# baajur/sda

Hardware: AMD Instinct MI355X
Metric: clerk share-combine GB/s + packed-Shamir shares/s at 1M-dim, 1/2/4/8 GPUs (higher is better)
Workload: dtype int64; 1 GPU; AdditiveSharing clerk combine, 10k participations x 1M-dim i64 shares per GPU (BASELINE.json configs[1]); participations_per_gpu=10000, dim=1000000, modulus=2147482801, parallelism=participation split x1, exact=combiner.rs:16-28 recurrence, bit-exact, buffers=torch.empty

## Files before the change

sda_amd/csrc/engine.cpp:

```cpp
#include "../../include/sda_engine.h"

#include <dlfcn.h>
#include <hip/hip_runtime.h>
#include <rccl/rccl.h>
#include <stdarg.h>
#include <stdio.h>
#include <stdlib.h>
#include <string.h>

#include <algorithm>
#include <map>
#include <mutex>
#include <string>
#include <thread>
#include <vector>

#include "host_pack.h"
#include "kernels.h"

struct sda_engine {
    int device = 0;
    hipStream_t stream = nullptr;
    void* work = nullptr;
    size_t work_bytes = 0;
    void* stage = nullptr;
    size_t stage_bytes = 0;
    sda::DeviceTable gen_tab;
    void* gen_log = nullptr;
    size_t gen_log_bytes = 0;
    bool gen_log_used = false;
    void* gen32_tmp = nullptr;
    size_t gen32_tmp_bytes = 0;
    void* codec_work = nullptr;
    size_t codec_work_bytes = 0;
    void* codec_mat = nullptr;
    size_t codec_mat_bytes = 0;
    void* pipe = nullptr;
    size_t pipe_bytes = 0;
    sda::DeviceTable rev_tab;
    void* snap = nullptr;
    size_t snap_bytes = 0;
    hipStream_t last_stream = nullptr;
    hipEvent_t order_ev = nullptr;
    bool order_ok = true;
    unsigned long long* rej_host = nullptr;
    hipStream_t copy_stream = nullptr;
    hipEvent_t h2d_done[2] = {nullptr, nullptr}, tile_free[2] = {nullptr, nullptr};
    void* hs_pin = nullptr;
    size_t hs_pin_bytes = 0;
    void* hs_dev = nullptr;
    size_t hs_dev_bytes = 0;
    uint64_t hs_tiles32 = 0, hs_tiles64 = 0, hs_bytes_h2d = 0;
    std::vector<sda_engine*> sub;
    void** comms = nullptr;
};

namespace {

thread_local std::string g_last_error;

thread_local sda_engine* t_call_h = nullptr;
thread_local hipStream_t t_call_s = nullptr;

void end_call() {
    if (t_call_h) {
        t_call_h->order_ok = hipEventRecord(t_call_h->order_ev, t_call_s) == hipSuccess;
        t_call_h = nullptr;
    }
}

thread_local int t_depth = 0;
struct CallScope {
    CallScope() { ++t_depth; }
    ~CallScope() {
        if (--t_depth == 0) end_call();
    }
    CallScope(const CallScope&) = delete;
    CallScope& operator=(const CallScope&) = delete;
};
#define SDA_ENTRY CallScope sda_call_scope_

sda_status fail(sda_status st, const char* fmt, ...) {
    char buf[512];
    va_list ap;
    va_start(ap, fmt);
    vsnprintf(buf, sizeof(buf), fmt, ap);
    va_end(ap);
    g_last_error = buf;
    return st;
}

sda_status ok() {
    g_last_error.clear();
    return SDA_OK;
}

#define HIP_TRY(expr)                                                                              \
    do {                                                                                           \
        hipError_t _e = (expr);                                                                    \
        if (_e != hipSuccess) {                                                                    \
            (void)hipGetLastError();                                                               \
            return fail(_e == hipErrorOutOfMemory ? SDA_ERR_OUT_OF_MEMORY : SDA_ERR_DEVICE,        \
                        "%s failed: %s (%s:%d)", #expr, hipGetErrorString(_e), __FILE__, __LINE__); \
        }                                                                                          \
    } while (0)

constexpr size_t kScratchHbmMin = (size_t)256 << 20;
bool scratch_hbm(size_t bytes) {
    static const bool on = [] {
        const char* e = getenv("SDA_SCRATCH_HBM");
        return e && atoi(e) == 1;
    }();
    return on && bytes >= kScratchHbmMin;
}
bool hbm_owned(void* p);
void hbm_engine_opened(int device);
bool hbm_engine_closed(int device);

void dev_free(void* p) {
    if (!p) return;
    if (hbm_owned(p)) (void)sda_hbm_free(p);
    else (void)hipFree(p);
}

sda_status dev_alloc(void** p, size_t bytes) {
    *p = nullptr;
    if (scratch_hbm(bytes)) {
        int d = 0;
        HIP_TRY(hipGetDevice(&d));
        return sda_hbm_alloc(d, bytes, p);
    }
    HIP_TRY(hipMalloc(p, bytes));
    return SDA_OK;
}

sda_status ensure(void** buf, size_t* have, size_t need) {
    if (need <= *have) return SDA_OK;
    dev_free(*buf);
    *buf = nullptr;
    *have = 0;
    size_t want = need + need / 4 + 4096;
    if (sda_status e = dev_alloc(buf, want)) return e;
    *have = want;
    return SDA_OK;
}

hipStream_t pick(sda_engine* h, void* stream) {
    hipStream_t s = static_cast<hipStream_t>(stream);
    if (s != h->last_stream) {
        if (!h->order_ok || hipStreamWaitEvent(s, h->order_ev, 0) != hipSuccess) (void)hipDeviceSynchronize();
        h->last_stream = s;
    }
    t_call_h = h;
    t_call_s = s;
    return s;
}

bool is_pow(uint64_t x, uint64_t b) {
    if (x < 1) return false;
    while (x % b == 0) x /= b;
    return x == 1;
}

// ... 1602 lines not shown
                                                static_cast<int64_t*>(h->hs_dev)))
            return e;
    }
    DevArena a;
    if (sda_status e = stage(h, rup(n_idx * share_len * 8 + 8) + rup(n_masks * width * 8 + 8) + rup(outn * 8 + 8), &a))
        return e;
    int64_t* dsh = a.take<int64_t>(n_idx * share_len + 1);
    void* dmask = a.take<int64_t>(n_masks * width + 1);
    int64_t* dout = a.take<int64_t>(outn + 1);
    for (uint64_t i = 0; i < n_idx; ++i)
        if (share_len) HIP_TRY(hipMemcpyAsync(dsh + i * share_len, share_rows[i], share_len * 8, hipMemcpyHostToDevice, h->stream));
    if (ms->kind == SDA_MASKING_FULL)
        for (uint64_t i = 0; i < n_masks; ++i)
            if (width) HIP_TRY(hipMemcpyAsync(static_cast<int64_t*>(dmask) + i * width, mask_rows[i], width * 8,
                                              hipMemcpyHostToDevice, h->stream));
    if (ms->kind == SDA_MASKING_CHACHA && !seeds.empty() && !multi_mask)
        HIP_TRY(hipMemcpyAsync(dmask, seeds.data(), seeds.size() * 4, hipMemcpyHostToDevice, h->stream));
    uint64_t len = 0;
    if (sda_status e = multi_mask
                           ? recipient_pipeline(h, &full_row, h->hs_dev, 1, ms->dimension, ss, dimension, indices, dsh,
                                                n_idx, share_len, output_modulus, mode, dout, (uint64_t)-1, &len, h->stream)
                           : recipient_pipeline(h, ms, dmask, n_masks, ms->kind == SDA_MASKING_NONE ? 0 : width, ss,
                                                dimension, indices, dsh, n_idx, share_len, output_modulus, mode, dout,
                                                (uint64_t)-1, &len, h->stream))
        return e;
    if (out_cap < len) return fail(SDA_ERR_INVALID_ARGUMENT, "output buffer too small");
    if (len) HIP_TRY(hipMemcpyAsync(out, dout, len * 8, hipMemcpyDeviceToHost, h->stream));
    *out_len = len;
    return finish(h);
}

sda_status sda_participant_share_dev(sda_engine* h, const sda_masking_scheme* ms, const uint32_t* seed,
                                     uint64_t seed_words, const int64_t* full_masks, const sda_sharing_scheme* ss,
                                     const int64_t* secrets, uint64_t dimension, const int64_t* draws,
                                     int32_t mode, int64_t* shares_out, uint8_t* payload, uint64_t payload_cap,
                                     uint64_t* payload_row_bytes, void* stream) {
    SDA_ENTRY;
    if (!h || !ms || !ss || (dimension && (!secrets || !shares_out)) || (payload && !payload_row_bytes))
        return fail(SDA_ERR_INVALID_ARGUMENT, "NULL argument");
    HIP_TRY(hipSetDevice(h->device));
    hipStream_t st = pick(h, stream);
    const uint64_t D = dimension;
    const bool packed = ss->kind == SDA_SHARING_PACKED_SHAMIR;
    if (!packed && ss->kind != SDA_SHARING_ADDITIVE) return fail(SDA_ERR_INVALID_ARGUMENT, "unknown sharing scheme kind");
    if (mode != SDA_REVEAL_EXACT && mode != SDA_REVEAL_CANONICAL) return fail(SDA_ERR_INVALID_ARGUMENT, "bad mode");
    if (packed) {
        if (sda_status e = check_packed(ss)) return e;
    } else {
        if (ss->share_count == 0) return fail(SDA_ERR_PRECONDITION, "share_count - 1 underflows (additive.rs:42)");
        if (ss->modulus <= 0) return fail(SDA_ERR_PRECONDITION, "Rng.gen_range called with low >= high");
    }
    const int64_t* masked = secrets;
    bool mask_pending = false;
    int64_t* cmask = nullptr;
    uint32_t* cseed = nullptr;
    uint32_t cw = 0;
    if (ms->kind != SDA_MASKING_NONE && D) {
        if (ms->modulus <= 0) return fail(SDA_ERR_PRECONDITION, "Rng.gen_range called with low >= high");
        if (sda_status e = ensure(&h->pipe, &h->pipe_bytes, 2 * rup(D * 8) + 256)) return e;
        int64_t* dm = static_cast<int64_t*>(h->pipe);
        if (ms->kind == SDA_MASKING_FULL) {
            if (!full_masks) return fail(SDA_ERR_INVALID_ARGUMENT, "Full masking needs the drawn masks");
            HIP_TRY(sda::launch_addsub_trem(secrets, full_masks, +1, D, dm, ms->modulus, st));
        } else if (ms->kind == SDA_MASKING_CHACHA) {
            if (ms->dimension != D) return fail(SDA_ERR_PRECONDITION, "assertion failed: dimension == secrets.len()");
            const uint64_t want = (ms->seed_bitsize + 31) / 32;
            if (seed_words != want || (seed_words && !seed))
                return fail(SDA_ERR_PRECONDITION, "expected %llu seed words", (unsigned long long)want);
            int64_t* dmask = dm + rup(D * 8) / 8;
            uint32_t* dseed = reinterpret_cast<uint32_t*>(dmask + rup(D * 8) / 8);
            const uint32_t w = (uint32_t)(seed_words < 8 ? seed_words : 8);
            if (w) HIP_TRY(hipMemcpyAsync(dseed, seed, w * 4, hipMemcpyHostToDevice, st));
            const char* force = getenv("SDA_CHACHA_PATH");
            if (!sda::chacha_needs_stream_path(ms->modulus) && !(force && strcmp(force, "stream") == 0)) {
                if (sda_status e = ensure(&h->work, &h->work_bytes, sda::chacha_work_bytes(D, 0))) return e;
                HIP_TRY(sda::launch_chacha_mask_add_async(ms->modulus, D, dseed, w, secrets, dm, h->work, st,
                                                          h->rej_host));
                mask_pending = true;
            } else {
                if (sda_status e = chacha_combine(h, ms->modulus, D, dseed, w, 1, dmask, st)) return e;
                HIP_TRY(sda::launch_addsub_trem(secrets, dmask, +1, D, dm, ms->modulus, st));
            }
            cmask = dmask;
            cseed = dseed;
            cw = w;
        } else {
            return fail(SDA_ERR_INVALID_ARGUMENT, "unknown masking scheme kind");
        }
        masked = dm;
    }
    const uint64_t n = ss->share_count;
    const uint64_t B = packed ? (D + ss->secret_count - 1) / ss->secret_count : D;
    if (B && !draws) return fail(SDA_ERR_INVALID_ARGUMENT, "need the randomness draws");
    if (payload && n > 65535) return fail(SDA_ERR_UNSUPPORTED, "at most 65535 clerks");
    auto share_and_encode = [&]() -> sda_status {
        if (B) {
            if (packed) {
                if (sda_status e = ensure(&h->gen_log, &h->gen_log_bytes, sda::packed_gen_log_bytes())) return e;
                sda::PackedGenArgs ga{masked, D, 1, draws, shares_out, mode == SDA_REVEAL_CANONICAL};
                HIP_TRY(sda::launch_packed_generate(ga, (uint32_t)ss->secret_count, (uint32_t)ss->privacy_threshold,
                                                    (uint32_t)n, (uint32_t)ss->modulus, (uint32_t)ss->omega_secrets,
                                                    (uint32_t)ss->omega_shares, h->gen_tab, h->gen_log, st,
                                                    &h->gen_log_used));
            } else {
                HIP_TRY(sda::launch_additive_generate(masked, D, draws, n, shares_out, ss->modulus, st));
            }
        }
        if (payload) {
            if (sda_status e = ensure(&h->codec_work, &h->codec_work_bytes, sda::varint_encode_work_bytes(n, B)))
                return e;
            hipError_t e = sda::launch_varint_encode(shares_out, n, B, B, payload, payload_cap, h->codec_work,
                                                     payload_row_bytes, st);
            if (e == hipErrorInvalidValue) return fail(SDA_ERR_INVALID_ARGUMENT, "payload_cap too small");
            HIP_TRY(e);
        }
        return SDA_OK;
    };
    if (sda_status e = share_and_encode()) return e;
    if (mask_pending) {
        HIP_TRY(hipStreamSynchronize(st));
        if (*h->rej_host) {
            if (sda_status e = chacha_combine(h, ms->modulus, D, cseed, cw, 1, cmask, st)) return e;
            HIP_TRY(sda::launch_addsub_trem(secrets, cmask, +1, D, const_cast<int64_t*>(masked), ms->modulus, st));
            if (sda_status e = share_and_encode()) return e;
        }
    }
    return ok();
}

}

namespace {

long long env_ll(const char* name, long long dflt) {
    const char* e = getenv(name);
    return e && *e ? atoll(e) : dflt;
}

int host_threads(size_t devices = 1) {
    const long long t = env_ll("SDA_HOST_THREADS", 0);
    if (t > 0) return (int)std::min<long long>(t, 1024);
    const unsigned hc = std::thread::hardware_concurrency();
    return (int)std::max<unsigned>(1u, std::min<unsigned>(hc ? hc : 1u, 16u * (unsigned)devices));
}

uint64_t host_stage_bytes() {
    const long long mb = env_ll("SDA_HOST_STAGE_MB", 256);
    return (uint64_t)std::max<long long>(mb, 1) << 20;
}

using sda::pack_rows;
using sda::pack_rows32;

bool host_narrow() { return env_ll("SDA_HOST_NARROW", 1) != 0; }

sda_status host_stream_ensure(sda_engine* h, size_t tile_bytes, size_t acc_bytes) {
    if (!h->copy_stream) {
        HIP_TRY(hipStreamCreateWithFlags(&h->copy_stream, hipStreamNonBlocking));
        for (int b = 0; b < 2; ++b) {
            HIP_TRY(hipEventCreateWithFlags(&h->h2d_done[b], hipEventDisableTiming));
            HIP_TRY(hipEventCreateWithFlags(&h->tile_free[b], hipEventDisableTiming));
        }
    }
    if (h->hs_pin_bytes < 2 * rup(tile_bytes)) {
        if (h->hs_pin) (void)hipHostFree(h->hs_pin);
        h->hs_pin = nullptr;
        h->hs_pin_bytes = 0;
        HIP_TRY(hipHostMalloc(&h->hs_pin, 2 * rup(tile_bytes), hipHostMallocDefault));
        h->hs_pin_bytes = 2 * rup(tile_bytes);
    }
    const size_t dev_need = 2 * rup(tile_bytes) + rup(acc_bytes);
    if (h->hs_dev_bytes < dev_need) {
        dev_free(h->hs_dev);
        h->hs_dev = nullptr;
        h->hs_dev_bytes = 0;
        if (sda_status e = dev_alloc(&h->hs_dev, dev_need)) return e;
        h->hs_dev_bytes = dev_need;
    }
    return SDA_OK;
}

sda_status stream_combine_slice(sda_engine* h, int64_t m, const int64_t* const* rows, uint64_t n_rows, uint64_t lo,
                                uint64_t w, int64_t* out_host, int threads) {
    HIP_TRY(hipSetDevice(h->device));
    const uint64_t stage = host_stage_bytes();
    const bool narrow = host_narrow();
    const uint64_t wc_max = std::max<uint64_t>(2, stage / 8 / 2 * 2);
    for (uint64_t c0 = 0; c0 < w; c0 += wc_max) {
        const uint64_t wc = std::min(wc_max, w - c0);
        const uint64_t R = std::max<uint64_t>(1, stage / (wc * 8));
        const size_t tile = (size_t)(std::min(R, std::max<uint64_t>(n_rows, 1)) * wc * 8);
        if (sda_status e = host_stream_ensure(h, tile, wc * 8)) return e;
        int64_t* dt[2] = {static_cast<int64_t*>(h->hs_dev), static_cast<int64_t*>(h->hs_dev) + rup(tile) / 8};
        int64_t* acc = static_cast<int64_t*>(h->hs_dev) + 2 * rup(tile) / 8;
        int64_t* hp[2] = {static_cast<int64_t*>(h->hs_pin), static_cast<int64_t*>(h->hs_pin) + rup(tile) / 8};
        uint64_t i = 0;
        bool try32 = narrow;
        for (uint64_t r0 = 0; r0 < n_rows; r0 += R, ++i) {
            const uint64_t Ri = std::min(R, n_rows - r0);
            const int b = (int)(i & 1);
            if (i >= 2) HIP_TRY(hipEventSynchronize(h->h2d_done[b]));
            if (try32) try32 = pack_rows32(reinterpret_cast<int32_t*>(hp[b]), rows, r0, Ri, lo + c0, wc, threads);
            if (!try32) pack_rows(hp[b], rows, r0, Ri, lo + c0, wc, threads);
            const size_t bytes = (size_t)(Ri * wc * (try32 ? 4 : 8));
            if (i >= 2) HIP_TRY(hipStreamWaitEvent(h->copy_stream, h->tile_free[b], 0));
            HIP_TRY(hipMemcpyAsync(dt[b], hp[b], bytes, hipMemcpyHostToDevice, h->copy_stream));
            HIP_TRY(hipEventRecord(h->h2d_done[b], h->copy_stream));
            HIP_TRY(hipStreamWaitEvent(h->stream, h->h2d_done[b], 0));
            if (try32)
                HIP_TRY(sda::launch_combine_wide32(reinterpret_cast<const int32_t*>(dt[b]), Ri, wc, wc, acc, m,
                                                   h->stream, i > 0));
            else
                HIP_TRY(sda::launch_combine_exact(dt[b], Ri, wc, wc, acc, m, h->stream, i > 0));
            HIP_TRY(hipEventRecord(h->tile_free[b], h->stream));
            ++(try32 ? h->hs_tiles32 : h->hs_tiles64);
            h->hs_bytes_h2d += bytes;
        }
        HIP_TRY(hipMemcpyAsync(out_host + c0, acc, wc * 8, hipMemcpyDeviceToHost, h->stream));
        HIP_TRY(hipStreamSynchronize(h->stream));
    }
    return SDA_OK;
}

size_t n_devices(const sda_engine* h) { return h->sub.empty() ? 1 : h->sub.size(); }

template <typename F>
sda_status for_devices(sda_engine* h, F fn) {
    const size_t G = n_devices(h);
    if (G == 1) return fn(0);
    std::vector<sda_status> st(G, SDA_OK);
    std::vector<std::string> msg(G);
    std::vector<std::thread> ts;
    for (size_t g = 1; g < G; ++g)
        ts.emplace_back([&, g] {
            st[g] = fn(g);
            if (st[g]) msg[g] = g_last_error;
        });
    st[0] = fn(0);
    if (st[0]) msg[0] = g_last_error;
    for (auto& t : ts) t.join();
    for (size_t g = 0; g < G; ++g)
        if (st[g]) return fail(st[g], "device %d: %s", h->sub[g]->device, msg[g].c_str());
    return SDA_OK;
}

void column_slice(uint64_t dim, size_t g, size_t G, uint64_t* lo, uint64_t* w) {
    const uint64_t pairs = (dim + 1) / 2, base = pairs / G, extra = pairs % G;
    const uint64_t start = g * base + std::min<uint64_t>(g, extra), count = base + (g < extra ? 1 : 0);
    *lo = std::min(dim, 2 * start);
    *w = std::min(dim, 2 * (start + count)) - *lo;
}

void shard(uint64_t n, size_t g, size_t G, uint64_t* start, uint64_t* count) {
    const uint64_t base = n / G, extra = n % G;
    *start = g * base + std::min<uint64_t>(g, extra);
    *count = base + (g < extra ? 1 : 0);
}

sda_engine* dev_of(sda_engine* h, size_t g) { return h->sub.empty() ? h : h->sub[g]; }

sda_status host_combine(sda_engine* h, int64_t m, const int64_t* const* rows, uint64_t n_rows, uint64_t dim,
                        int64_t* out) {
    const size_t G = n_devices(h);
    const int T = std::max(1, host_threads(G) / (int)G);
    return for_devices(h, [&](size_t g) -> sda_status {
        uint64_t lo, w;
        column_slice(dim, g, G, &lo, &w);
        if (w == 0) return SDA_OK;
        return stream_combine_slice(dev_of(h, g), m, rows, n_rows, lo, w, out + lo, T);
    });
}

struct Rccl {
    bool ok = false;
    std::string err;
    ncclResult_t (*comm_init_all)(ncclComm_t*, int, const int*) = nullptr;
    ncclResult_t (*comm_destroy)(ncclComm_t) = nullptr;
    ncclResult_t (*reduce)(const void*, void*, size_t, ncclDataType_t, ncclRedOp_t, int, ncclComm_t,
                           hipStream_t) = nullptr;
    ncclResult_t (*group_start)() = nullptr;
    ncclResult_t (*group_end)() = nullptr;
    const char* (*error_string)(ncclResult_t) = nullptr;
};

Rccl& rccl() {
    static Rccl r;
    static std::once_flag once;
    std::call_once(once, [] {
        void* lib = dlopen("librccl.so.1", RTLD_NOW | RTLD_LOCAL);
        if (!lib) {
            r.err = dlerror() ? dlerror() : "dlopen(librccl.so.1) failed";
            return;
        }
        r.comm_init_all = reinterpret_cast<decltype(r.comm_init_all)>(dlsym(lib, "ncclCommInitAll"));
        r.comm_destroy = reinterpret_cast<decltype(r.comm_destroy)>(dlsym(lib, "ncclCommDestroy"));
        r.reduce = reinterpret_cast<decltype(r.reduce)>(dlsym(lib, "ncclReduce"));
        r.group_start = reinterpret_cast<decltype(r.group_start)>(dlsym(lib, "ncclGroupStart"));
        r.group_end = reinterpret_cast<decltype(r.group_end)>(dlsym(lib, "ncclGroupEnd"));
        r.error_string = reinterpret_cast<decltype(r.error_string)>(dlsym(lib, "ncclGetErrorString"));
        r.ok = r.comm_init_all && r.comm_destroy && r.reduce && r.group_start && r.group_end && r.error_string;
        if (!r.ok) r.err = "librccl.so.1 lacks an entry point";
    });
    return r;
}

#define NCCL_TRY(expr)                                                                                  \
    do {                                                                                                \
        ncclResult_t _r = (expr);                                                                       \
        if (_r != ncclSuccess)                                                                          \
            return fail(SDA_ERR_DEVICE, "%s failed: %s (%s:%d)", #expr, rccl().error_string(_r), __FILE__, \
                        __LINE__);                                                                      \
    } while (0)

bool distinct_devices(const sda_engine* h) {
    for (size_t a = 0; a < h->sub.size(); ++a)
        for (size_t b = a + 1; b < h->sub.size(); ++b)
            if (h->sub[a]->device == h->sub[b]->device) return false;
    return true;
}

sda_status ensure_comms(sda_engine* h) {
    if (h->comms) return SDA_OK;
    Rccl& r = rccl();
    if (!r.ok) return fail(SDA_ERR_DEVICE, "RCCL unavailable: %s", r.err.c_str());
    const size_t G = n_devices(h);
    std::vector<int> devs(G);
    for (size_t g = 0; g < G; ++g) devs[g] = dev_of(h, g)->device;
    std::vector<ncclComm_t> comms(G, nullptr);
    NCCL_TRY(r.comm_init_all(comms.data(), (int)G, devs.data()));
    h->comms = new void*[G];
    for (size_t g = 0; g < G; ++g) h->comms[g] = comms[g];
    return SDA_OK;
}

void destroy_comms(sda_engine* h) {
    if (!h->comms) return;
    for (size_t g = 0; g < n_devices(h); ++g)
        if (h->comms[g]) (void)rccl().comm_destroy(static_cast<ncclComm_t>(h->comms[g]));
    delete[] h->comms;
    h->comms = nullptr;
}

sda_status chacha_combine_multi(sda_engine* h, int64_t m, uint64_t D, const std::vector<uint32_t>& seeds, uint32_t w,
                                uint64_t n, int64_t* dst) {
    const size_t G = n_devices(h);
    const bool split = !h->sub.empty() && distinct_devices(h) && n >= G && !sda::chacha_needs_stream_path(m) &&
                       (unsigned __int128)G * (uint64_t)(m - 1) <= (unsigned __int128)INT64_MAX;
    const size_t parts = split ? G : 1;
    std::vector<int64_t*> partial(parts, nullptr);
    sda_status st = for_devices(h, [&](size_t g) -> sda_status {
        if (g >= parts) return SDA_OK;
        sda_engine* d = dev_of(h, g);
        HIP_TRY(hipSetDevice(d->device));
        uint64_t s0 = 0, cnt = n;
        if (split) shard(n, g, G, &s0, &cnt);
        DevArena a;
        if (sda_status e = stage(d, rup(cnt * w * 4 + 4) + rup(D * 8), &a)) return e;
        uint32_t* dseeds = a.take<uint32_t>(cnt * w + 1);
        partial[g] = split ? a.take<int64_t>(D) : dst;
        if (cnt) HIP_TRY(hipMemcpyAsync(dseeds, seeds.data() + s0 * w, cnt * w * 4, hipMemcpyHostToDevice, d->stream));
        return chacha_combine(d, m, D, dseeds, w, cnt, partial[g], d->stream);
    });
    if (st) return st;
    HIP_TRY(hipSetDevice(h->device));
    if (!split) return SDA_OK;
    if (sda_status e = ensure_comms(h)) return e;
    Rccl& r = rccl();
    NCCL_TRY(r.group_start());
    for (size_t g = 0; g < G; ++g) {
        sda_engine* d = dev_of(h, g);
        ncclResult_t rr = r.reduce(partial[g], partial[g], D, ncclInt64, ncclSum, 0,
                                   static_cast<ncclComm_t>(h->comms[g]), d->stream);
        if (rr != ncclSuccess) {
            (void)r.group_end();
            return fail(SDA_ERR_DEVICE, "ncclReduce: %s", r.error_string(rr));
        }
    }
    NCCL_TRY(r.group_end());
    HIP_TRY(hipSetDevice(h->device));
    HIP_TRY(sda::launch_mod_canonical(partial[0], D, dst, m, h->stream));
    for (size_t g = 1; g < G; ++g) HIP_TRY(hipStreamSynchronize(dev_of(h, g)->stream));
    return SDA_OK;
}

sda_status host_chacha_combine(sda_engine* h, int64_t m, uint64_t D, const std::vector<uint32_t>& seeds, uint32_t w,
                               uint64_t n, int64_t* out_host) {
    HIP_TRY(hipSetDevice(h->device));
    if (sda_status e = host_stream_ensure(h, 0, D * 8)) return e;
    int64_t* dst = static_cast<int64_t*>(h->hs_dev);
    if (sda_status e = chacha_combine_multi(h, m, D, seeds, w, n, dst)) return e;
    HIP_TRY(hipMemcpyAsync(out_host, dst, D * 8, hipMemcpyDeviceToHost, h->stream));
    HIP_TRY(hipStreamSynchronize(h->stream));
    return SDA_OK;
}

sda_status host_decode_combine(sda_engine* h, int64_t m, const uint8_t* const* blobs, const uint64_t* lens, uint64_t n,
                               int64_t* out, uint64_t out_cap, uint64_t* out_len) {
    *out_len = 0;
    if (n == 0) return SDA_OK;
    const uint64_t stage = host_stage_bytes();
    struct Group { uint64_t b0, nb, bytes; };
    std::vector<Group> groups;
    for (uint64_t i = 0; i < n;) {
        Group g{i, 0, 0};
        while (i < n && (g.nb == 0 || g.bytes + lens[i] <= stage)) g.bytes += lens[i++], ++g.nb;
        groups.push_back(g);
    }
    uint64_t biggest = 0;
    for (auto& g : groups) biggest = std::max(biggest, g.bytes);
    const size_t slot = rup(biggest + 32);
    if (sda_status e = host_stream_ensure(h, slot, 0)) return e;
    uint8_t* hp[2] = {static_cast<uint8_t*>(h->hs_pin), static_cast<uint8_t*>(h->hs_pin) + rup(slot)};
    uint8_t* dbytes[2] = {static_cast<uint8_t*>(h->hs_dev), static_cast<uint8_t*>(h->hs_dev) + rup(slot)};
    const int T = host_threads();
    auto pack = [&](const Group& g, uint8_t* dst, std::vector<uint64_t>* off) {
        off->assign(g.nb + 1, 0);
        for (uint64_t i = 0; i < g.nb; ++i) (*off)[i + 1] = (*off)[i] + lens[g.b0 + i];
        std::vector<std::thread> ts;
        const uint64_t per = (g.nb + T - 1) / T;
        for (int t = 0; t < T && (uint64_t)t * per < g.nb; ++t)
            ts.emplace_back([&, t] {
                for (uint64_t i = (uint64_t)t * per; i < g.nb && i < (uint64_t)(t + 1) * per; ++i)
// ... 176 lines not shown
```

sda_amd/csrc/host_pack.h:

```cpp
#pragma once
#include <limits.h>
#include <stdint.h>
#include <string.h>

#include <algorithm>
#include <atomic>
#include <thread>
#include <vector>

namespace sda {

namespace host_pack_detail {

template <typename F>
void split_elements(uint64_t total, int threads, F work) {
    const uint64_t min_per_thread = 512 * 1024;
    const int T = (int)std::max<uint64_t>(1, std::min<uint64_t>((uint64_t)threads, total / min_per_thread));
    if (T <= 1) {
        work(0, total);
        return;
    }
    const uint64_t per = (total + T - 1) / T;
    std::vector<std::thread> ts;
    ts.reserve(T - 1);
    for (int t = 1; t < T; ++t) {
        const uint64_t e0 = std::min(total, (uint64_t)t * per), e1 = std::min(total, e0 + per);
        if (e0 < e1) ts.emplace_back(work, e0, e1);
    }
    work(0, std::min(per, total));
    for (auto& t : ts) t.join();
}

inline const unsigned char* row_at(const int64_t* row, uint64_t c) {
    return reinterpret_cast<const unsigned char*>(row) + c * 8;
}

}

inline void pack_rows(int64_t* dst, const int64_t* const* rows, uint64_t r0, uint64_t R, uint64_t lo, uint64_t w,
                      int threads) {
    const uint64_t total = R * w;
    auto work = [=](uint64_t e0, uint64_t e1) {
        while (e0 < e1) {
            const uint64_t r = e0 / w, c = e0 % w;
            const uint64_t n = std::min(e1 - e0, w - c);
            memcpy(dst + e0, host_pack_detail::row_at(rows[r0 + r], lo + c), n * 8);
            e0 += n;
        }
    };
    host_pack_detail::split_elements(total, threads, work);
}

inline bool pack_rows32(int32_t* dst, const int64_t* const* rows, uint64_t r0, uint64_t R, uint64_t lo, uint64_t w,
                        int threads) {
    const uint64_t total = R * w;
    std::atomic<bool> wide(false);
    std::atomic<bool>* const wp = &wide;
    auto work = [=](uint64_t e0, uint64_t e1) {
        while (e0 < e1 && !wp->load(std::memory_order_relaxed)) {
            const uint64_t r = e0 / w, c = e0 % w;
            const uint64_t n = std::min(e1 - e0, w - c);
            const unsigned char* src = host_pack_detail::row_at(rows[r0 + r], lo + c);
            int32_t* d = dst + e0;
            uint64_t bad = 0;
            for (uint64_t i = 0; i < n; ++i) {
                int64_t v;
                memcpy(&v, src + i * 8, 8);
                const int32_t t = (int32_t)(uint32_t)(uint64_t)v;
                bad |= (uint64_t)(v ^ (int64_t)t);
                d[i] = t;
            }
            if (bad) {
                wp->store(true, std::memory_order_relaxed);
                return;
            }
            e0 += n;
        }
    };
    host_pack_detail::split_elements(total, threads, work);
    return !wide.load();
}

}
```

Measured before the change: 6682 GB/s.

## Reuse persistent pack thread pool and vectorize int64-to-int32 narrowing with AVX2

Replaces per-tile thread spawn/join in host row packing with a persistent condition-variable worker pool created once per device slice. It also adds an AVX2 narrowing body that deinterleaves low and high 32-bit halves, checks that the values fit, and writes to pinned staging memory with non-temporal stores followed by an sfence. The goal is to cut thread-creation overhead and speed up the CPU pack that feeds host-to-device uploads. It adds optional stderr tracing of pack and wait times and an env switch back to the scalar path. The pool's synchronization adds complexity.

```diff
diff --git a/sda_amd/csrc/engine.cpp b/sda_amd/csrc/engine.cpp
--- a/sda_amd/csrc/engine.cpp
+++ b/sda_amd/csrc/engine.cpp
@@ -9,6 +9,7 @@
 #include <string.h>
 
 #include <algorithm>
+#include <chrono>
 #include <map>
 #include <mutex>
 #include <string>
@@ -1917,6 +1918,12 @@
 using sda::pack_rows;
 using sda::pack_rows32;
 
+bool host_trace() { return env_ll("SDA_HOST_TRACE", 0) != 0; }
+
+double seconds_since(std::chrono::steady_clock::time_point t0) {
+    return std::chrono::duration<double>(std::chrono::steady_clock::now() - t0).count();
+}
+
 bool host_narrow() { return env_ll("SDA_HOST_NARROW", 1) != 0; }
 
 sda_status host_stream_ensure(sda_engine* h, size_t tile_bytes, size_t acc_bytes) {
@@ -1946,10 +1953,15 @@
 }
 
 sda_status stream_combine_slice(sda_engine* h, int64_t m, const int64_t* const* rows, uint64_t n_rows, uint64_t lo,
-                                uint64_t w, int64_t* out_host, int threads) {
+                                uint64_t w, int64_t* out_host, sda::PackPool& pool) {
     HIP_TRY(hipSetDevice(h->device));
     const uint64_t stage = host_stage_bytes();
     const bool narrow = host_narrow();
+    const sda::PackBody body = sda::pack_body();
+    const bool trace = host_trace();
+    const auto t_call = std::chrono::steady_clock::now();
+    double pack_s = 0, wait_s = 0;
+    uint64_t n32 = 0, n64 = 0, chunks = 0, tile_rows = 0, tile_cols = 0;
     const uint64_t wc_max = std::max<uint64_t>(2, stage / 8 / 2 * 2);
     for (uint64_t c0 = 0; c0 < w; c0 += wc_max) {
         const uint64_t wc = std::min(wc_max, w - c0);
@@ -1964,9 +1976,14 @@
         for (uint64_t r0 = 0; r0 < n_rows; r0 += R, ++i) {
             const uint64_t Ri = std::min(R, n_rows - r0);
             const int b = (int)(i & 1);
+            auto t0 = std::chrono::steady_clock::now();
             if (i >= 2) HIP_TRY(hipEventSynchronize(h->h2d_done[b]));
-            if (try32) try32 = pack_rows32(reinterpret_cast<int32_t*>(hp[b]), rows, r0, Ri, lo + c0, wc, threads);
-            if (!try32) pack_rows(hp[b], rows, r0, Ri, lo + c0, wc, threads);
+            wait_s += seconds_since(t0);
+            t0 = std::chrono::steady_clock::now();
+            if (try32) try32 = pack_rows32(pool, reinterpret_cast<int32_t*>(hp[b]), rows, r0, Ri, lo + c0, wc, body);
+            if (!try32) pack_rows(pool, hp[b], rows, r0, Ri, lo + c0, wc);
+            pack_s += seconds_since(t0);
+            ++(try32 ? n32 : n64);
             const size_t bytes = (size_t)(Ri * wc * (try32 ? 4 : 8));
             if (i >= 2) HIP_TRY(hipStreamWaitEvent(h->copy_stream, h->tile_free[b], 0));
             HIP_TRY(hipMemcpyAsync(dt[b], hp[b], bytes, hipMemcpyHostToDevice, h->copy_stream));
@@ -1983,7 +2000,18 @@
         }
         HIP_TRY(hipMemcpyAsync(out_host + c0, acc, wc * 8, hipMemcpyDeviceToHost, h->stream));
         HIP_TRY(hipStreamSynchronize(h->stream));
-    }
+        if (c0 == 0) tile_rows = std::min(R, n_rows), tile_cols = wc;
+        ++chunks;
+    }
+    if (trace)
+        fprintf(stderr,
+                "[sda host trace] device %d: %llu rows x %llu columns, tiles %llu int32 + %llu i64 of %llu rows x %llu "
+                "columns in %llu column chunk(s), %d pack thread(s), %s body: pack %.4f s, blocked on upload %.4f s, "
+                "total %.4f s\n",
+                h->device, (unsigned long long)n_rows, (unsigned long long)w, (unsigned long long)n32,
+                (unsigned long long)n64, (unsigned long long)tile_rows, (unsigned long long)tile_cols,
+                (unsigned long long)chunks, pool.threads(), body == sda::PackBody::Avx2 ? "avx2" : "scalar", pack_s,
+                wait_s, seconds_since(t_call));
     return SDA_OK;
 }
 
@@ -2032,7 +2060,8 @@
         uint64_t lo, w;
         column_slice(dim, g, G, &lo, &w);
         if (w == 0) return SDA_OK;
-        return stream_combine_slice(dev_of(h, g), m, rows, n_rows, lo, w, out + lo, T);
+        sda::PackPool pool(T);
+        return stream_combine_slice(dev_of(h, g), m, rows, n_rows, lo, w, out + lo, pool);
     });
 }
 
diff --git a/sda_amd/csrc/host_pack.h b/sda_amd/csrc/host_pack.h
--- a/sda_amd/csrc/host_pack.h
+++ b/sda_amd/csrc/host_pack.h
@@ -1,44 +1,167 @@
 #pragma once
 #include <limits.h>
 #include <stdint.h>
+#include <stdlib.h>
 #include <string.h>
 
 #include <algorithm>
 #include <atomic>
+#include <condition_variable>
+#include <mutex>
 #include <thread>
 #include <vector>
 
+#if defined(__x86_64__) && !defined(__HIP_DEVICE_COMPILE__)
+#include <immintrin.h>
+#define SDA_HOST_PACK_X86 1
+#endif
+
 namespace sda {
 
+enum class PackBody { Scalar, Avx2 };
+
+constexpr uint64_t kPackMinPerThread = 512 * 1024;
+
 namespace host_pack_detail {
-
-template <typename F>
-void split_elements(uint64_t total, int threads, F work) {
-    const uint64_t min_per_thread = 512 * 1024;
-    const int T = (int)std::max<uint64_t>(1, std::min<uint64_t>((uint64_t)threads, total / min_per_thread));
-    if (T <= 1) {
-        work(0, total);
-        return;
-    }
-    const uint64_t per = (total + T - 1) / T;
-    std::vector<std::thread> ts;
-    ts.reserve(T - 1);
-    for (int t = 1; t < T; ++t) {
-        const uint64_t e0 = std::min(total, (uint64_t)t * per), e1 = std::min(total, e0 + per);
-        if (e0 < e1) ts.emplace_back(work, e0, e1);
-    }
-    work(0, std::min(per, total));
-    for (auto& t : ts) t.join();
-}
 
 inline const unsigned char* row_at(const int64_t* row, uint64_t c) {
     return reinterpret_cast<const unsigned char*>(row) + c * 8;
 }
 
-}
-
-inline void pack_rows(int64_t* dst, const int64_t* const* rows, uint64_t r0, uint64_t R, uint64_t lo, uint64_t w,
-                      int threads) {
+inline uint64_t narrow_scalar(int32_t* d, const unsigned char* src, uint64_t n) {
+    uint64_t bad = 0;
+    for (uint64_t i = 0; i < n; ++i) {
+        int64_t v;
+        memcpy(&v, src + i * 8, 8);
+        const int32_t t = (int32_t)(uint32_t)(uint64_t)v;
+        bad |= (uint64_t)(v ^ (int64_t)t);
+        d[i] = t;
+    }
+    return bad;
+}
+
+#ifdef SDA_HOST_PACK_X86
+inline bool cpu_has_avx2() {
+    static const bool has = __builtin_cpu_supports("avx2");
+    return has;
+}
+
+__attribute__((target("avx2"))) inline uint64_t narrow_avx2(int32_t* d, const unsigned char* src, uint64_t n) {
+    const uintptr_t a = reinterpret_cast<uintptr_t>(d);
+    if (a & 3) return narrow_scalar(d, src, n);
+    const uint64_t head = std::min<uint64_t>(n, ((32 - (a & 31)) & 31) / 4);
+    uint64_t bad = narrow_scalar(d, src, head);
+    uint64_t i = head;
+    __m256i vbad = _mm256_setzero_si256();
+    for (; i + 8 <= n; i += 8) {
+        const __m256 x = _mm256_loadu_ps(reinterpret_cast<const float*>(src + i * 8));
+        const __m256 y = _mm256_loadu_ps(reinterpret_cast<const float*>(src + i * 8 + 32));
+        const __m256i lo = _mm256_castps_si256(_mm256_shuffle_ps(x, y, 0x88));
+        const __m256i hi = _mm256_castps_si256(_mm256_shuffle_ps(x, y, 0xDD));
+        vbad = _mm256_or_si256(vbad, _mm256_xor_si256(hi, _mm256_srai_epi32(lo, 31)));
+        _mm256_stream_si256(reinterpret_cast<__m256i*>(d + i), _mm256_permute4x64_epi64(lo, 0xD8));
+    }
+    bad |= (uint64_t)!_mm256_testz_si256(vbad, vbad);
+    return bad | narrow_scalar(d + i, src + i * 8, n - i);
+}
+
+inline void stream_fence() { _mm_sfence(); }
+#else
+inline bool cpu_has_avx2() { return false; }
+inline uint64_t narrow_avx2(int32_t* d, const unsigned char* src, uint64_t n) { return narrow_scalar(d, src, n); }
+inline void stream_fence() {}
+#endif
+
+}
+
+inline bool pack_body_supported(PackBody body) {
+    return body == PackBody::Scalar || host_pack_detail::cpu_has_avx2();
+}
+
+inline PackBody pack_body() {
+    const char* e = getenv("SDA_HOST_PACK");
+    if (e && strcmp(e, "scalar") == 0) return PackBody::Scalar;
+    return host_pack_detail::cpu_has_avx2() ? PackBody::Avx2 : PackBody::Scalar;
+}
+
+class PackPool {
+public:
+    explicit PackPool(int threads) : threads_(std::max(1, threads)) {}
+    PackPool(const PackPool&) = delete;
+    PackPool& operator=(const PackPool&) = delete;
+    ~PackPool() {
+        {
+            std::lock_guard<std::mutex> lk(mu_);
+            stop_ = true;
+        }
+        wake_.notify_all();
+        for (auto& t : workers_) t.join();
+    }
+
+    int threads() const { return threads_; }
+
+    template <typename F>
+    void run(uint64_t total, uint64_t min_per_thread, const F& work) {
+        const int T = (int)std::max<uint64_t>(
+            1, std::min<uint64_t>((uint64_t)threads_, total / std::max<uint64_t>(1, min_per_thread)));
+        if (T <= 1) {
+            work(0, total);
+            return;
+        }
+        const uint64_t per = (total + T - 1) / T;
+        while ((int)workers_.size() < T - 1) {
+            const int id = (int)workers_.size() + 1;
+            const uint64_t seen = gen_;
+            workers_.emplace_back([this, id, seen] { worker(id, seen); });
+        }
+        {
+            std::lock_guard<std::mutex> lk(mu_);
+            fn_ = [](const void* f, uint64_t e0, uint64_t e1) { (*static_cast<const F*>(f))(e0, e1); };
+            arg_ = &work;
+            total_ = total;
+            per_ = per;
+            pending_ = 0;
+            for (int t = 1; t < T; ++t) pending_ += (uint64_t)t * per < total;
+            active_ = T;
+            ++gen_;
+        }
+        wake_.notify_all();
+        work(0, std::min(per, total));
+        std::unique_lock<std::mutex> lk(mu_);
+        done_.wait(lk, [this] { return pending_ == 0; });
+    }
+
+private:
+    void worker(int id, uint64_t seen) {
+        std::unique_lock<std::mutex> lk(mu_);
+        for (;;) {
+            wake_.wait(lk, [&] { return stop_ || gen_ != seen; });
+            if (gen_ == seen) return;
+            seen = gen_;
+            const uint64_t e0 = (uint64_t)id * per_, e1 = std::min(total_, e0 + per_);
+            if (id >= active_ || e0 >= total_) continue;
+            auto fn = fn_;
+            const void* arg = arg_;
+            lk.unlock();
+            fn(arg, e0, e1);
+            lk.lock();
+            if (--pending_ == 0) done_.notify_one();
+        }
+    }
+
+    const int threads_;
+    std::vector<std::thread> workers_;
+    std::mutex mu_;
+    std::condition_variable wake_, done_;
+    void (*fn_)(const void*, uint64_t, uint64_t) = nullptr;
+    const void* arg_ = nullptr;
+    uint64_t total_ = 0, per_ = 0, gen_ = 0;
+    int active_ = 0, pending_ = 0;
+    bool stop_ = false;
+};
+
+inline void pack_rows(PackPool& pool, int64_t* dst, const int64_t* const* rows, uint64_t r0, uint64_t R,
+                      uint64_t lo, uint64_t w, uint64_t min_per_thread = kPackMinPerThread) {
     const uint64_t total = R * w;
     auto work = [=](uint64_t e0, uint64_t e1) {
         while (e0 < e1) {
@@ -48,12 +171,13 @@
             e0 += n;
         }
     };
-    host_pack_detail::split_elements(total, threads, work);
-}
-
-inline bool pack_rows32(int32_t* dst, const int64_t* const* rows, uint64_t r0, uint64_t R, uint64_t lo, uint64_t w,
-                        int threads) {
+    pool.run(total, min_per_thread, work);
+}
+
+inline bool pack_rows32(PackPool& pool, int32_t* dst, const int64_t* const* rows, uint64_t r0, uint64_t R,
+                        uint64_t lo, uint64_t w, PackBody body, uint64_t min_per_thread = kPackMinPerThread) {
     const uint64_t total = R * w;
+    const bool avx2 = body == PackBody::Avx2 && host_pack_detail::cpu_has_avx2();
     std::atomic<bool> wide(false);
     std::atomic<bool>* const wp = &wide;
     auto work = [=](uint64_t e0, uint64_t e1) {
@@ -61,24 +185,30 @@
             const uint64_t r = e0 / w, c = e0 % w;
             const uint64_t n = std::min(e1 - e0, w - c);
             const unsigned char* src = host_pack_detail::row_at(rows[r0 + r], lo + c);
-            int32_t* d = dst + e0;
-            uint64_t bad = 0;
-            for (uint64_t i = 0; i < n; ++i) {
-                int64_t v;
-                memcpy(&v, src + i * 8, 8);
-                const int32_t t = (int32_t)(uint32_t)(uint64_t)v;
-                bad |= (uint64_t)(v ^ (int64_t)t);
-                d[i] = t;
-            }
+            const uint64_t bad = avx2 ? host_pack_detail::narrow_avx2(dst + e0, src, n)
+                                      : host_pack_detail::narrow_scalar(dst + e0, src, n);
             if (bad) {
                 wp->store(true, std::memory_order_relaxed);
-                return;
+                break;
             }
             e0 += n;
         }
+        if (avx2) host_pack_detail::stream_fence();
     };
-    host_pack_detail::split_elements(total, threads, work);
+    pool.run(total, min_per_thread, work);
     return !wide.load();
 }
 
-}
+inline void pack_rows(int64_t* dst, const int64_t* const* rows, uint64_t r0, uint64_t R, uint64_t lo, uint64_t w,
+                      int threads) {
+    PackPool pool(threads);
+    pack_rows(pool, dst, rows, r0, R, lo, w);
+}
+
+inline bool pack_rows32(int32_t* dst, const int64_t* const* rows, uint64_t r0, uint64_t R, uint64_t lo, uint64_t w,
+                        int threads) {
+    PackPool pool(threads);
+    return pack_rows32(pool, dst, rows, r0, R, lo, w, pack_body());
+}
+
+}
```

Measured after the change: 6681 GB/s. Within noise of the previous version (-0.0%).
